# iris1997jiatong/I-DCCRN-VAE

Hardware: AMD Instinct MI355X
Metric: 4s@16kHz utterances/sec fwd+SI-SNR, DCCRN-CL, 1/2/4/8 MI355X vs host CPU (higher is better)
Workload: dtype f32; 1 GPU; supervised DCCRN-CL forward(train=False) + final_ete_loss (weights 0/0/1); batch_per_gpu=64, utterance=4 s @ 16 kHz (64000 samples, 641 frames), parallelism=replicas x1, streams=1, input=resident in HBM

## Files before the change

i-dccrn-vae_amd/csrc/cgemm_tw.hip:

```cpp
#include <atomic>
#include <cstdint>
#include <cstdlib>
#include <type_traits>
#include "cgemm.hpp"
#include "../../include/idccrn_hip.h"

namespace {

struct TwArgs {
    const float* x0;
    const float* x1;
    int C0, C1;
    int Fin, Fout;
    int J, Jp, Tp;
    const float* wfrag;
    int UP;
    const float* epi;
    int has_fold;
    const float* slope;
    float* out;
    int Cout, cotiles;
    int tshift, t_valid;
    double* stats;
    int stats_rep;
    const float* add;
    int add_div, add_Jp;
    int jtiles, ftiles;
    int xcd_split;
    int cgroups;
    int stagger;
};

constexpr int TW_PACK_CI = 8;
constexpr int TW_WVEC_MASK = 1;
constexpr int TW_XCD_SPLIT = 1;
constexpr int TW_PAIR_STAGGER = 1;

template <int PH> __device__ __forceinline__ int tw_ra(int r) {
    if (PH == 0) return r == 0 ? 0 : (r == 2 ? 2 : 1);
    return r == 0 ? 1 : 2;
}
template <int PH> __device__ __forceinline__ int tw_rb(int r) {
    if (PH == 0) return r == 2 ? 1 : (r == 3 ? 3 : 2);
    return r == 0 ? 2 : 3;
}
template <int PH> __device__ __forceinline__ float tw_cb(int r) {
    if (PH == 0) return r == 1 ? 1.f : -1.f;
    return r == 1 ? 0.f : -1.f;
}
template <int PH> constexpr int tw_nr() { return PH == 0 ? 4 : 3; }
template <int PH> constexpr int tw_nt() { return tw_nr<PH>() * 9; }
template <int PH> constexpr int tw_ntp() { return PH == 0 ? 36 : 32; }
template <int PH> constexpr int tw_ntw() { return (tw_nt<PH>() + 3) / 4; }
__host__ __device__ inline int tw_tile(int ph, int w, int k) {
    if (ph == 0) return w * 9 + k;
    if (w < 3) return k < 6 ? w * 9 + k : w * 9 + 8;
    return k < 6 ? (k >> 1) * 9 + 6 + (k & 1) : -1;
}
template <int PH> constexpr int tw_wslots() { return PH == 0 ? 9 : 8; }

template <int PH, int CIK, bool LEFT, bool STATS = false, int NCT = 1>
__global__ __launch_bounds__(256 * NCT, NCT == 1 ? 2 : 1) void cconv_tw_kernel(const TwArgs a) {
    constexpr int NR = tw_nr<PH>(), NT = tw_nt<PH>(), NTP = tw_ntp<PH>(), NTW = tw_ntw<PH>();
    constexpr int NRAW = PH == 0 ? 4 : 3, ROW0 = PH == 0 ? 0 : 1;
    constexpr int KS = CIK / 2;
    constexpr int RT = NRAW * 9 * 32;
    constexpr int NE = CIK * RT;
    constexpr int NBUF = 2;
    constexpr int RDW = 2;
    constexpr bool WVEC = (TW_WVEC_MASK >> PH) & 1;
    constexpr int NITEM = CIK * NRAW * 16;
    constexpr int NTHR = 256 * NCT;
    constexpr int NLD = (NITEM + NTHR - 1) / NTHR;
    static_assert(NCT == 1 || NCT == 2, "one or two co tiles per workgroup");
    static_assert(KS % RDW == 0 && NLD <= 2, "weight ring slots are compile-time; at most two staging items per thread");
    static_assert(NLD + NCT - 1 < KS, "the staging k-steps (from 1 on, waves 4 .. 7 one later) end before the barrier's k-step");
    static_assert(NCT * NT * 4 * 64 <= NBUF * NE, "the epilogue exchange (one area per co tile) fits the patch buffers");

    extern __shared__ __attribute__((aligned(16))) float smem[];

    const int tid = threadIdx.x;
    const int lane = tid & 63;
    const int wave = __builtin_amdgcn_readfirstlane(tid >> 6);
    const int w4 = NCT == 1 ? wave : wave & 3, cth = NCT == 1 ? 0 : wave >> 2;
    const int half = lane >> 5, l31 = lane & 31;

    const int bid = blockIdx.x;
    const int xcd = bid & 7, slot = bid >> 3;
    int jt, ft, ct;
    if (a.xcd_split) {
        const int G = 8 / a.cgroups;
        ct = xcd % a.cgroups;
        jt = (slot / a.ftiles) * G + xcd / a.cgroups;
        ft = slot - (slot / a.ftiles) * a.ftiles;
    } else {
        const int per = a.cgroups * a.ftiles;
        jt = (slot / per) * 8 + xcd;
        const int rem = slot - (slot / per) * per;
        ft = rem / a.cgroups;
        ct = rem - ft * a.cgroups;
    }
    if (jt >= a.jtiles) return;
    ct = NCT * ct + cth;
    const int j0 = jt * 64;
    const int m0 = 2 * ft;
    const int rbase = m0 - 1 + ROW0;

    const int Cin = a.C0 + a.C1;
    const int nchunk = (Cin + CIK - 1) / CIK;

    f32x16 acc[NTW];
#pragma unroll
    for (int k = 0; k < NTW; ++k)
#pragma unroll
        for (int r = 0; r < 16; ++r) acc[k][r] = 0.f;
    constexpr int NPAIR = (NTW - 1) / 2;
    constexpr bool UNI = PH == 0;
    int offA[UNI ? 1 : NPAIR + 1], offB[UNI ? 1 : NPAIR + 1];
    float cbj[UNI ? 1 : NPAIR + 1];
    if (UNI) {
        cbj[0] = tw_cb<PH>(w4);
        offA[0] = (tw_ra<PH>(w4) - ROW0) * 288;
        offB[0] = (tw_rb<PH>(w4) - ROW0) * 288;
    } else {
#pragma unroll
        for (int j = 0; j <= NPAIR; ++j) {
            int t = tw_tile(PH, w4, j < NPAIR ? 2 * j : NTW - 1);
            t = t < 0 ? 0 : t;
            const int r = t / 9, plane = t - r * 9;
            cbj[j] = tw_cb<PH>(r);
            const int po = plane == 8 ? 256 : (plane >> 1) * 64;
            offA[j] = (tw_ra<PH>(r) - ROW0) * 288 + po;
            offB[j] = cbj[j] != 0.f ? (tw_rb<PH>(r) - ROW0) * 288 + po : offA[j];
        }
    }

    f32x4 v_r[NLD], v_i[NLD];
    float e_r[NLD], e_i[NLD];
    unsigned off_v[NLD], off_e[NLD], ldsoff[NLD];
    unsigned okmask[NLD];
    int item_cl[NLD];
    bool interior[NLD];
#pragma unroll
    for (int i = 0; i < NLD; ++i) {
        const int e = tid + i * NTHR;
        const int c8 = e & 15;
        const int rl = (e >> 4) % NRAW, cl = e / (16 * NRAW);
        item_cl[i] = cl;
        const int f = rbase + rl;
        const int jc = j0 + 4 * c8;
        const int je = LEFT ? jc - 1 : jc + 4;
        const bool exists = e < NITEM;
        const bool okr = exists && f >= 0 && f < a.Fin;
        unsigned m = 0;
#pragma unroll
        for (int q = 0; q < 5; ++q) {
            const int c = jc + q + (LEFT ? -1 : 0);
            if (c >= 0 && c < a.J) m |= 1u << q;
        }
        if (okr) m |= 1u << 5;
        if (exists) m |= 1u << 7;
        const int jcv = jc + 3 < a.Jp ? jc : 0;
        const int jev = (je >= 0 && je < a.Jp) ? je : 0;
        off_v[i] = okr ? (unsigned)((cl * a.Fin + f) * a.Jp + jcv) : 0u;
        off_e[i] = okr ? (unsigned)((cl * a.Fin + f) * a.Jp + jev) : 0u;
        if (jc + 3 >= a.Jp) m &= ~0x1fu;
        if (!(je >= 0 && je < a.Jp)) m &= LEFT ? ~1u : ~(1u << 4);
        okmask[i] = m;
        interior[i] = __builtin_amdgcn_ballot_w64((m & 0xbfu) == 0xbfu) == ~0ull;
        ldsoff[i] = (unsigned)((cl * NRAW + rl) * 288 + 4 * c8);
    }
    auto stage_load = [&](int chunk, int i) {
        const int ci0 = chunk * CIK;
        const bool from0 = ci0 < a.C0;
        const float* br = from0 ? a.x0 + (size_t)ci0 * a.Fin * a.Jp : a.x1 + (size_t)(ci0 - a.C0) * a.Fin * a.Jp;
        const float* bi = from0 ? br + (size_t)a.C0 * a.Fin * a.Jp : br + (size_t)a.C1 * a.Fin * a.Jp;
        const int cvalid = (from0 ? a.C0 : Cin) - ci0;
        const bool dead = item_cl[i] >= cvalid;
        const unsigned ov = dead ? 0u : off_v[i], oe = dead ? 0u : off_e[i];
        v_r[i] = *(const f32x4*)(br + ov);
        v_i[i] = *(const f32x4*)(bi + ov);
        e_r[i] = br[oe];
        e_i[i] = bi[oe];
    };
    float fr[5], fi[5];
    auto stage_window = [&](int chunk, int i) {
        const int ci0s = chunk * CIK;
        const int cvalid = (ci0s < a.C0 ? a.C0 : Cin) - ci0s;
        constexpr bool left = LEFT;
        if (interior[i] && cvalid >= CIK) {
#pragma unroll
            for (int q = 0; q < 5; ++q) {
                fr[q] = left ? (q == 0 ? e_r[i] : v_r[i][q == 0 ? 0 : q - 1]) : (q == 4 ? e_r[i] : v_r[i][q == 4 ? 3 : q]);
                fi[q] = left ? (q == 0 ? e_i[i] : v_i[i][q == 0 ? 0 : q - 1]) : (q == 4 ? e_i[i] : v_i[i][q == 4 ? 3 : q]);
            }
            return;
        }
        unsigned m = okmask[i];
        if (item_cl[i] >= cvalid || !((m >> 5) & 1u)) m &= ~0x1fu;
#pragma unroll
        for (int q = 0; q < 5; ++q) {
            const float xr = left ? (q == 0 ? e_r[i] : v_r[i][q == 0 ? 0 : q - 1]) : (q == 4 ? e_r[i] : v_r[i][q == 4 ? 3 : q]);
            const float xi = left ? (q == 0 ? e_i[i] : v_i[i][q == 0 ? 0 : q - 1]) : (q == 4 ? e_i[i] : v_i[i][q == 4 ? 3 : q]);
            const bool cok = (m >> q) & 1u;
            fr[q] = cok ? xr : 0.f;
            fi[q] = cok ? xi : 0.f;
        }
    };
    auto plane_val = [&](int gt, int pr) -> float {
        const int g = gt / 3, tau = gt - g * 3;
        const int q0 = 2 * pr;
        const float xa_ = g == 0 ? fr[q0] + fi[q0] : (g == 1 ? fr[q0] : fi[q0]);
        const float xb_ = g == 0 ? fr[q0 + 1] + fi[q0 + 1] : (g == 1 ? fr[q0 + 1] : fi[q0 + 1]);
        const float xd_ = g == 0 ? fr[q0 + 2] + fi[q0 + 2] : (g == 1 ? fr[q0 + 2] : fi[q0 + 2]);
        return tau == 0 ? xa_ - xb_ : (tau == 1 ? xb_ : xb_ - xd_);
    };
    auto item_exists = [&](int i) -> bool { return NITEM >= (i + 1) * NTHR || wave * 64 + i * NTHR < NITEM; };
    auto stage_plane2 = [&](float* dst, int i, int j) {
        if (!item_exists(i)) return;
        if (j < 4) {
            f32x4 o = {plane_val(2 * j, 0), plane_val(2 * j + 1, 0), plane_val(2 * j, 1), plane_val(2 * j + 1, 1)};
            *(f32x4*)(dst + ldsoff[i] + j * 64) = o;
        } else {
            *(float2*)(dst + ldsoff[i] - 2 * (int)(tid & 15) + 256) = make_float2(plane_val(8, 0), plane_val(8, 1));
        }
    };
    auto stage_store = [&](float* dst, int chunk, int i) {
        stage_window(chunk, i);
#pragma unroll
        for (int j = 0; j < 5; ++j) stage_plane2(dst, i, j);
    };

    constexpr int WS = tw_wslots<PH>();
    const float* wbase = a.wfrag + ((size_t)(PH == 1 ? (size_t)a.cotiles * a.UP * tw_ntp<0>() : 0) + (size_t)ct * a.UP * NTP) * 64 +
                         (size_t)w4 * WS * 64;
    const int total_ks = nchunk * KS;
    float a_w[RDW][NTW];
    auto load_w = [&](int g, float (&dst)[NTW]) {
        g = g < total_ks ? g : total_ks - 1;
        const float* ws = wbase + (size_t)g * NTP * 64;
        if (WVEC) {
            const f32x4 w0 = *(const f32x4*)(ws + lane * 4), w1 = *(const f32x4*)(ws + 256 + lane * 4);
#pragma unroll
            for (int k = 0; k < 4; ++k) {
                dst[k] = w0[k];
                if (4 + k < NTW) dst[4 + k] = w1[k];
            }
            if (NTW == 9) dst[NTW - 1] = ws[512 + lane];
        } else {
#pragma unroll
            for (int k = 0; k < NTW; ++k) dst[k] = ws[k * 64 + lane];
        }
    };
    float xa[NTW], xb[NTW];
    auto load_raw2 = [&](const float* base, int j) {
        if (j < NPAIR) {
            const int oa = UNI ? offA[0] + j * 64 : offA[UNI ? 0 : j], ob = UNI ? offB[0] + j * 64 : offB[UNI ? 0 : j];
            const float2 pa_ = *(const float2*)(base + oa + 2 * l31), pb_ = *(const float2*)(base + ob + 2 * l31);
            xa[2 * j] = pa_.x; xa[2 * j + 1] = pa_.y;
            xb[2 * j] = pb_.x; xb[2 * j + 1] = pb_.y;
        } else {
            xa[NTW - 1] = base[(UNI ? offA[0] + 256 : offA[UNI ? 0 : NPAIR]) + l31];
            xb[NTW - 1] = base[(UNI ? offB[0] + 256 : offB[UNI ? 0 : NPAIR]) + l31];
        }
    };
    auto load_raw_all = [&](const float* base) {
#pragma unroll
        for (int j = 0; j <= NPAIR; ++j) load_raw2(base, j);
    };

#pragma unroll
    for (int i = 0; i < NLD; ++i) stage_load(0, i);
#pragma unroll
    for (int u = 0; u < RDW; ++u) load_w(u, a_w[u]);
#pragma unroll
    for (int i = 0; i < NLD; ++i) stage_store(smem, 0, i);
#pragma unroll
    for (int i = 0; i < NLD; ++i) stage_load(nchunk > 1 ? 1 : 0, i);
    __syncthreads();

    load_raw_all(smem + (size_t)half * RT);
    auto run = [&](auto late_) {
        constexpr bool LATE = decltype(late_)::value;
        for (int chunk = 0; chunk < nchunk; ++chunk) {
            const float* P = smem + (chunk & 1) * NE;
            float* Pn = smem + ((chunk + 1) & 1) * NE;
            const int nxt = chunk + 1 < nchunk ? chunk + 1 : chunk, nxt2 = chunk + 2 < nchunk ? chunk + 2 : nchunk - 1;
#pragma unroll
            for (int ul = 0; ul < KS; ++ul) {
                const float* bnext = ul + 1 < KS ? P + (size_t)(2 * (ul + 1) + half) * RT : Pn + (size_t)half * RT;
                const int si = ul - 1 - (LATE ? 1 : 0);
                const bool staging = si >= 0 && si < NLD;
#pragma unroll
                for (int k = 0; k < NTW; ++k) {
                    const float b = xa[k] + cbj[UNI ? 0 : (k >> 1 < NPAIR ? k >> 1 : NPAIR)] * xb[k];
                    acc[k] = __builtin_amdgcn_mfma_f32_32x32x2f32(a_w[ul % RDW][k], b, acc[k], 0, 0, 0);
                    if (ul == KS - 1 && k == 0) {
                        __builtin_amdgcn_sched_barrier(0);
                        __syncthreads();
                    }
                    if ((k & 1) && (k >> 1) < NPAIR) load_raw2(bnext, k >> 1);
                    if (k == NTW - 1) load_raw2(bnext, NPAIR);
                    if (staging) {
                        if (k == 0) stage_window(nxt, si);
                        if ((k & 1) && k < 6) stage_plane2(Pn, si, k >> 1);
                        if (k == (NTW == 9 ? 7 : 6)) stage_plane2(Pn, si, 3);
                        if (k == NTW - 1) stage_plane2(Pn, si, 4);
                        if (k == NTW - 1) stage_load(nxt2, si);
                    }
                    __builtin_amdgcn_sched_barrier(0);
                }
                load_w(chunk * KS + ul + RDW, a_w[ul % RDW]);
            }
        }
    };
    if (NCT == 2 && PH == 1 && a.stagger && cth)
        run(std::integral_constant<bool, NCT == 2 && PH == 1>{});
    else
        run(std::false_type{});
    __syncthreads();

    const float slope = a.slope ? *a.slope : 1.0f;
    const bool has_act = a.slope != nullptr;
    float* E = smem + cth * (NT * 4 * 64);
    const int jA = j0 + 2 * l31;
    bool keep[2], inb[2];
    int ja[2];
#pragma unroll
    for (int q = 0; q < 2; ++q) {
        const int j = jA + q;
        const int bj = j / a.Tp, tp = j - bj * a.Tp;
        inb[q] = j < a.J;
        keep[q] = inb[q] && tp >= 1 && tp <= a.t_valid;
        ja[q] = j - (bj - bj / a.add_div) * a.Tp;
    }
#pragma unroll
    for (int s = 0; s < 4; ++s) {
        if (s > 0) __syncthreads();
#pragma unroll
        for (int k = 0; k < NTW; ++k) {
            const int t = tw_tile(PH, w4, k);
            if (t >= 0) {
#pragma unroll
                for (int rr = 0; rr < 4; ++rr) E[(t * 4 + rr) * 64 + lane] = acc[k][4 * s + rr];
            }
        }
        __syncthreads();
        float v[NT];
#pragma unroll
        for (int t = 0; t < NT; ++t) v[t] = E[(t * 4 + w4) * 64 + lane];
        float pr[NR][2], pi[NR][2];
#pragma unroll
        for (int r = 0; r < NR; ++r) {
            float y[3][2];
#pragma unroll
            for (int g = 0; g < 3; ++g) {
                const float m1 = v[r * 9 + g * 3], m2 = v[r * 9 + g * 3 + 1], m3 = v[r * 9 + g * 3 + 2];
                y[g][0] = m1 + m2;
                y[g][1] = m2 - m3;
            }
#pragma unroll
            for (int q = 0; q < 2; ++q) {
                pr[r][q] = y[0][q] - y[2][q];
                pi[r][q] = y[0][q] + y[1][q];
            }
        }
        const int rg = 4 * s + w4;
        const int co = ct * 32 + (rg & 3) + 8 * (rg >> 2) + 4 * half;
        const bool cok = co < a.Cout;
        const f32x4 e0 = *(const f32x4*)(a.epi + (size_t)co * 8);
        const float e4 = a.epi[(size_t)co * 8 + 4], e5 = a.epi[(size_t)co * 8 + 5];
        float st[5] = {0.f, 0.f, 0.f, 0.f, 0.f};
#pragma unroll
        for (int rt = 0; rt < 2; ++rt) {
            const int fo = 2 * m0 + PH + 2 * rt;
            if (fo >= a.Fout) continue;
            float yr[2], yi[2];
#pragma unroll
            for (int q = 0; q < 2; ++q) {
                float re, im;
                if (PH == 0) {
                    re = rt == 0 ? pr[0][q] + pr[1][q] + pr[2][q] : pr[1][q] - pr[2][q] - pr[NR - 1][q];
                    im = rt == 0 ? pi[0][q] + pi[1][q] + pi[2][q] : pi[1][q] - pi[2][q] - pi[NR - 1][q];
                } else {
                    re = rt == 0 ? pr[0][q] + pr[1][q] : pr[1][q] - pr[2][q];
                    im = rt == 0 ? pi[0][q] + pi[1][q] : pi[1][q] - pi[2][q];
                }
                if (a.add && cok && inb[q]) {
                    re += a.add[((size_t)co * a.Fout + fo) * a.add_Jp + ja[q]];
                    im += a.add[((size_t)(a.Cout + co) * a.Fout + fo) * a.add_Jp + ja[q]];
                }
                float r_, i_;
                if (a.has_fold) {
                    r_ = e0[0] * re + e0[1] * im + e4;
                    i_ = e0[2] * re + e0[3] * im + e5;
                } else {
                    r_ = re + e4;
                    i_ = im + e5;
                }
                if (has_act) {
                    r_ = r_ >= 0.f ? r_ : slope * r_;
                    i_ = i_ >= 0.f ? i_ : slope * i_;
                }
                yr[q] = keep[q] ? r_ : 0.f;
                yi[q] = keep[q] ? i_ : 0.f;
                if (STATS && keep[q]) {
                    st[0] += yr[q];
                    st[1] += yi[q];
                    st[2] += yr[q] * yr[q];
                    st[3] += yi[q] * yi[q];
                    st[4] += yr[q] * yi[q];
                }
            }
            if (cok) {
                float* o_r = a.out + ((size_t)co * a.Fout + fo) * a.Jp + jA;
                float* o_i = a.out + ((size_t)(a.Cout + co) * a.Fout + fo) * a.Jp + jA;
                if (inb[1]) {
                    *(float2*)o_r = make_float2(yr[0], yr[1]);
                    *(float2*)o_i = make_float2(yi[0], yi[1]);
                } else if (inb[0]) {
                    o_r[0] = yr[0];
                    o_i[0] = yi[0];
                }
            }
        }
        if (STATS) {
#pragma unroll
            for (int q = 0; q < 5; ++q) {
                float tsum = st[q];
#pragma unroll
                for (int o = 16; o > 0; o >>= 1) tsum += __shfl_xor(tsum, o, 64);
                if (l31 == 0 && cok)
                    atomicAdd(&a.stats[((size_t)(a.stats_rep > 1 ? (blockIdx.x & (a.stats_rep - 1)) : 0) * a.Cout + co) * 5 + q], (double)tsum);
            }
        }
    }
}

__global__ void pack_cconv_tw_kernel(const float* __restrict__ wino, int cotiles, int UN, int UP, int vec, float* __restrict__ out) {
    const long long n0 = (long long)cotiles * UP * tw_ntp<0>() * 64, n1 = (long long)cotiles * UP * tw_ntp<1>() * 64;
    for (long long idx = blockIdx.x * (long long)blockDim.x + threadIdx.x; idx < n0 + n1; idx += (long long)gridDim.x * blockDim.x) {
        const int ph = idx >= n0;
        const long long i = ph ? idx - n0 : idx;
        const int ntp = ph ? tw_ntp<1>() : tw_ntp<0>(), nt = ph ? tw_nt<1>() : tw_nt<0>();
        const int lane = (int)(i & 63);
        long long t_ = i >> 6;
        const int t = (int)(t_ % ntp); t_ /= ntp;
        const int u = (int)(t_ % UP);
        const int ct = (int)(t_ / UP);
        float val = 0.f;
        const int ws_ = ph ? tw_wslots<1>() : tw_wslots<0>();
        const int pos = t * 64 + lane, w = pos / (ws_ * 64), q = pos % (ws_ * 64);
        const bool vec_ = (vec >> ph) & 1;
        const int k = !vec_ ? q >> 6 : (q < 512 ? (q >> 8) * 4 + (q & 3) : 8);
        const int ln = !vec_ ? q & 63 : (q < 512 ? (q & 255) >> 2 : q - 512);
        const int tt = k < (ph ? 7 : 9) ? tw_tile(ph, w, k) : -1;
        const int ci = 2 * u + (ln >> 5), co = ln & 31;
        if (tt >= 0 && ci * 3 < UN) {
            const int r = tt / 9, g = (tt % 9) / 3, tau = tt % 3;
            const float* src = wino + ((((size_t)ph * cotiles + ct) * UN + (size_t)ci * 3 + g) * 4 + r) * 64;
            const float w0 = src[co], w1 = src[32 + co];
            val = tau == 0 ? w0 : (tau == 1 ? w0 + w1 : w1);
        }
        out[idx] = val;
    }
}

template <int PH, int CIK, bool LEFT, bool STATS, int NCT>
int launch_tw_ph_l(const TwArgs& a, hipStream_t st) {
    constexpr int NE = CIK * (PH == 0 ? 4 : 3) * 9 * 32;
    constexpr size_t smem = 2 * NE * sizeof(float);
    static_assert(smem * (NCT == 1 ? 2 : 1) <= 160 * 1024, "the patch buffers of two workgroups (NCT = 2: of one) must fit the 160 KB of LDS");
    TwArgs b = a;
    b.jtiles = (a.J + 63) / 64;
    b.ftiles = PH == 1 ? a.Fin / 2 : (a.Fin + 1) / 2;
    if (b.ftiles == 0) return IDV_OK;
    b.cgroups = b.cotiles / NCT;
    if (b.cgroups * NCT != b.cotiles) return IDV_EINVAL;
    b.stagger = TW_PAIR_STAGGER;
    b.xcd_split = (TW_XCD_SPLIT && (b.cgroups == 2 || b.cgroups == 4 || b.cgroups == 8)) ? 1 : 0;
    long long nblk = (long long)((b.jtiles + 7) / 8) * 8 * b.ftiles * b.cgroups;
    if (b.xcd_split) {
        const int G = 8 / b.cgroups;
        nblk = (long long)((b.jtiles + G - 1) / G) * b.ftiles * 8;
    }
    if (nblk > 0x7fffffffLL) return IDV_EINVAL;
    auto k = cconv_tw_kernel<PH, CIK, LEFT, STATS, NCT>;
    static std::atomic<bool> attr_set[64];
    int dev = 0;
    if (hipGetDevice(&dev) != hipSuccess || dev < 0 || dev >= 64) return IDV_ELAUNCH;
    if (smem > 64 * 1024 && !attr_set[dev].load(std::memory_order_acquire)) {
        if (hipFuncSetAttribute((const void*)k, hipFuncAttributeMaxDynamicSharedMemorySize, (int)smem) != hipSuccess) return IDV_ELAUNCH;
        attr_set[dev].store(true, std::memory_order_release);
    }
    hipLaunchKernelGGL(k, dim3((unsigned)nblk), dim3(256 * NCT), smem, st, b);
    if (NCT > 1) idv_tw_pair_note_launch();
    return idv_launch_status();
}

template <int PH, int CIK>
int launch_tw_ph(const TwArgs& a, hipStream_t st) {
    const bool pair = a.cotiles % 2 == 0 && ((idv_tw_pair(-1) >> PH) & 1);
    switch ((a.stats ? 4 : 0) | (pair ? 2 : 0) | (a.tshift ? 1 : 0)) {
        case 0: return launch_tw_ph_l<PH, CIK, false, false, 1>(a, st);
        case 1: return launch_tw_ph_l<PH, CIK, true, false, 1>(a, st);
        case 2: return launch_tw_ph_l<PH, CIK, false, false, 2>(a, st);
        case 3: return launch_tw_ph_l<PH, CIK, true, false, 2>(a, st);
        case 4: return launch_tw_ph_l<PH, CIK, false, true, 1>(a, st);
        case 5: return launch_tw_ph_l<PH, CIK, true, true, 1>(a, st);
        case 6: return launch_tw_ph_l<PH, CIK, false, true, 2>(a, st);
        default: return launch_tw_ph_l<PH, CIK, true, true, 2>(a, st);
    }
}

}

namespace {
std::atomic<int>& tw_pair_mask() {
    static std::atomic<int> v{[] { const char* e = getenv("IDV_TW_PAIR"); return e ? atoi(e) & IDV_TW_PAIR_ALL : IDV_TW_PAIR_DEFAULT; }()};
    return v;
}
std::atomic<long long> tw_pair_launches{0};
}
void idv_tw_pair_note_launch() { tw_pair_launches.fetch_add(1, std::memory_order_relaxed); }
extern "C" int idv_tw_pair(int mask) {
    if (mask < 0) return tw_pair_mask().load(std::memory_order_relaxed);
    return tw_pair_mask().exchange(mask & IDV_TW_PAIR_ALL, std::memory_order_relaxed);
}
extern "C" long long idv_tw_pair_launches(int reset) {
    return reset ? tw_pair_launches.exchange(0, std::memory_order_relaxed) : tw_pair_launches.load(std::memory_order_relaxed);
}

extern "C" int idv_cconv_tw_supported(int C0, int C1, int Cout, int Fin) {
    static const int min_cout = [] { const char* e = getenv("IDV_TW_MIN_COUT"); return e ? atoi(e) : 32; }();
    if (Cout < min_cout || Fin < 2) return 0;
    if (!idv_cconv_gauss_supported(C0, C1, Cout)) return 0;
    return (C1 == 0 || C0 % 8 == 0) ? 1 : 0;
}

extern "C" long long idv_cconv_tw_wfrag_floats(int Cout, int cin_used) {
    const long long cotiles = (Cout + 31) / 32, cpad = (cin_used + TW_PACK_CI - 1) / TW_PACK_CI * TW_PACK_CI;
    return cotiles * (cpad / 2) * (36 + 32) * 64;
}

extern "C" int idv_pack_cconv_tw(const float* wino_frag, int Cout, int cin_used, float* tw_frag, void* stream) {
    if (!wino_frag || !tw_frag || Cout <= 0 || cin_used <= 0) return IDV_EINVAL;
    const int cotiles = (Cout + 31) / 32;
    const int cpad = (cin_used + TW_PACK_CI - 1) / TW_PACK_CI * TW_PACK_CI;
    const long long n = idv_cconv_tw_wfrag_floats(Cout, cin_used);
    const unsigned blocks = (unsigned)((n + 255) / 256 > 4096 ? 4096 : (n + 255) / 256);
    hipLaunchKernelGGL(pack_cconv_tw_kernel, dim3(blocks), dim3(256), 0, (hipStream_t)stream, wino_frag, cotiles, cpad * 3, cpad / 2,
                       TW_WVEC_MASK, tw_frag);
    return idv_launch_status();
}

extern "C" int idv_ctconv2d_tw_fwd(const float* x0, int C0, const float* x1, int C1, const float* wfrag, const float* epi, int has_fold,
                                   const float* prelu_slope, float* out, double* stats, double* stats_work, int stats_rep, int tshift,
                                   int Cout, int Fin, int B, int Tp, int Jp, int t_valid_out, const float* addend, int addend_div,
                                   int addend_Jp, void* stream) {
    if (!x0 || !wfrag || !epi || !out || C0 <= 0 || Cout <= 0 || Fin <= 0 || B <= 0 || Tp <= 1) return IDV_EINVAL;
    if (stats && stats_work && (stats_rep < 2 || (stats_rep & (stats_rep - 1)))) return IDV_EINVAL;
    if (addend && (addend_div < 1 || B % addend_div || addend_Jp < (B / addend_div) * Tp)) return IDV_EINVAL;
    if (C1 > 0 && !x1) return IDV_EINVAL;
    if (tshift != 0 && tshift != -1) return IDV_EINVAL;
    if (!idv_cconv_tw_supported(C0, C1, Cout, Fin)) return IDV_EINVAL;
    if ((Jp & 3) || (reinterpret_cast<uintptr_t>(x0) & 15) || (C1 > 0 && (reinterpret_cast<uintptr_t>(x1) & 15)) ||
        (reinterpret_cast<uintptr_t>(out) & 7))
        return IDV_EINVAL;
    TwArgs a{};
    a.x0 = x0; a.x1 = x1; a.C0 = C0; a.C1 = C1;
    a.Fin = Fin; a.Fout = 2 * Fin - 1;
    a.J = B * Tp; a.Jp = Jp; a.Tp = Tp;
    a.wfrag = wfrag; a.UP = (C0 + C1 + TW_PACK_CI - 1) / TW_PACK_CI * TW_PACK_CI / 2;
    a.epi = epi; a.has_fold = has_fold; a.slope = prelu_slope; a.out = out;
    a.Cout = Cout; a.cotiles = (Cout + 31) / 32;
    a.tshift = tshift; a.t_valid = t_valid_out;
    a.add = addend; a.add_div = addend ? addend_div : 1; a.add_Jp = addend_Jp;
    if (Jp < a.J) return IDV_EINVAL;
    if ((long long)8 * Fin * (long long)Jp >= 0xffffffffLL) return IDV_EINVAL;
    hipStream_t st = (hipStream_t)stream;
    a.stats = stats;
    if (stats && stats_work) { a.stats = stats_work; a.stats_rep = stats_rep; }
    int rc = 0;
    rc = launch_tw_ph<0, 8>(a, st);
    if (!rc) rc = launch_tw_ph<1, 8>(a, st);
    if (rc || !(stats && stats_work)) return rc;
    return idv_launch_stats_collapse(stats_work, stats_rep, Cout * 5, stats, st);
}
```

Baseline: 951.9 utterances/sec.

## Handle odd-Fin edge row with dedicated edge tiles in transposed complex conv

Result: faster. 973.7 utterances/sec (median of 6 runs) (+2.3%).

```diff
diff --git a/i-dccrn-vae_amd/csrc/cgemm_tw.hip b/i-dccrn-vae_amd/csrc/cgemm_tw.hip
--- a/i-dccrn-vae_amd/csrc/cgemm_tw.hip
+++ b/i-dccrn-vae_amd/csrc/cgemm_tw.hip
@@ -3,6 +3,7 @@
 #include <cstdlib>
 #include <type_traits>
 #include "cgemm.hpp"
+#include "cgemm_tw_map.hpp"
 #include "../../include/idccrn_hip.h"
 
 namespace {
@@ -25,9 +26,7 @@
     int stats_rep;
     const float* add;
     int add_div, add_Jp;
-    int jtiles, ftiles;
-    int xcd_split;
-    int cgroups;
+    TwGrid grid;
     int stagger;
 };
 
@@ -85,22 +84,11 @@
     const int w4 = NCT == 1 ? wave : wave & 3, cth = NCT == 1 ? 0 : wave >> 2;
     const int half = lane >> 5, l31 = lane & 31;
 
-    const int bid = blockIdx.x;
-    const int xcd = bid & 7, slot = bid >> 3;
-    int jt, ft, ct;
-    if (a.xcd_split) {
-        const int G = 8 / a.cgroups;
-        ct = xcd % a.cgroups;
-        jt = (slot / a.ftiles) * G + xcd / a.cgroups;
-        ft = slot - (slot / a.ftiles) * a.ftiles;
-    } else {
-        const int per = a.cgroups * a.ftiles;
-        jt = (slot / per) * 8 + xcd;
-        const int rem = slot - (slot / per) * per;
-        ft = rem / a.cgroups;
-        ct = rem - ft * a.cgroups;
-    }
-    if (jt >= a.jtiles) return;
+    TwTile tile;
+    if (!tw_block_tile(a.grid, blockIdx.x, tile)) return;
+    const bool edge = PH == 0 && tile.edge;
+    const int jt = tile.jt, ft = tile.ft;
+    int ct = tile.ct;
     ct = NCT * ct + cth;
     const int j0 = jt * 64;
     const int m0 = 2 * ft;
@@ -119,9 +107,9 @@
     int offA[UNI ? 1 : NPAIR + 1], offB[UNI ? 1 : NPAIR + 1];
     float cbj[UNI ? 1 : NPAIR + 1];
     if (UNI) {
-        cbj[0] = tw_cb<PH>(w4);
-        offA[0] = (tw_ra<PH>(w4) - ROW0) * 288;
-        offB[0] = (tw_rb<PH>(w4) - ROW0) * 288;
+        cbj[0] = edge ? 0.f : tw_cb<PH>(w4);
+        offA[0] = (edge ? w4 : tw_ra<PH>(w4) - ROW0) * 288;
+        offB[0] = (edge ? w4 : tw_rb<PH>(w4) - ROW0) * 288;
     } else {
 #pragma unroll
         for (int j = 0; j <= NPAIR; ++j) {
@@ -147,8 +135,8 @@
         const int c8 = e & 15;
         const int rl = (e >> 4) % NRAW, cl = e / (16 * NRAW);
         item_cl[i] = cl;
-        const int f = rbase + rl;
-        const int jc = j0 + 4 * c8;
+        const int f = edge ? a.Fin - 2 + (rl & 1) : rbase + rl;
+        const int jc = j0 + (edge ? 64 * (rl >> 1) : 0) + 4 * c8;
         const int je = LEFT ? jc - 1 : jc + 4;
         const bool exists = e < NITEM;
         const bool okr = exists && f >= 0 && f < a.Fin;
@@ -232,8 +220,8 @@
     };
 
     constexpr int WS = tw_wslots<PH>();
-    const float* wbase = a.wfrag + ((size_t)(PH == 1 ? (size_t)a.cotiles * a.UP * tw_ntp<0>() : 0) + (size_t)ct * a.UP * NTP) * 64 +
-                         (size_t)w4 * WS * 64;
+    const size_t wregion = PH == 1 ? (size_t)a.cotiles * a.UP * tw_ntp<0>() : (edge ? (size_t)a.cotiles * a.UP * (tw_ntp<0>() + tw_ntp<1>()) : 0);
+    const float* wbase = a.wfrag + (wregion + (size_t)ct * a.UP * NTP) * 64 + (size_t)w4 * WS * 64;
     const int total_ks = nchunk * KS;
     float a_w[RDW][NTW];
     auto load_w = [&](int g, float (&dst)[NTW]) {
@@ -323,17 +311,19 @@
     const float slope = a.slope ? *a.slope : 1.0f;
     const bool has_act = a.slope != nullptr;
     float* E = smem + cth * (NT * 4 * 64);
-    const int jA = j0 + 2 * l31;
-    bool keep[2], inb[2];
-    int ja[2];
-#pragma unroll
-    for (int q = 0; q < 2; ++q) {
-        const int j = jA + q;
-        const int bj = j / a.Tp, tp = j - bj * a.Tp;
-        inb[q] = j < a.J;
-        keep[q] = inb[q] && tp >= 1 && tp <= a.t_valid;
-        ja[q] = j - (bj - bj / a.add_div) * a.Tp;
-    }
+    const int jAc[2] = {j0 + 2 * l31, j0 + 2 * l31 + (edge ? 64 : 0)};
+    bool keep[2][2], inb[2][2];
+    int ja[2][2];
+#pragma unroll
+    for (int c = 0; c < 2; ++c)
+#pragma unroll
+        for (int q = 0; q < 2; ++q) {
+            const int j = jAc[c] + q;
+            const int bj = j / a.Tp, tp = j - bj * a.Tp;
+            inb[c][q] = j < a.J;
+            keep[c][q] = inb[c][q] && tp >= 1 && tp <= a.t_valid;
+            ja[c][q] = j - (bj - bj / a.add_div) * a.Tp;
+        }
 #pragma unroll
     for (int s = 0; s < 4; ++s) {
         if (s > 0) __syncthreads();
@@ -373,7 +363,8 @@
         float st[5] = {0.f, 0.f, 0.f, 0.f, 0.f};
 #pragma unroll
         for (int rt = 0; rt < 2; ++rt) {
-            const int fo = 2 * m0 + PH + 2 * rt;
+            const int fo = edge ? a.Fout - 1 : 2 * m0 + PH + 2 * rt;
+            const int jA = jAc[rt];
             if (fo >= a.Fout) continue;
             float yr[2], yi[2];
 #pragma unroll
@@ -382,13 +373,17 @@
                 if (PH == 0) {
                     re = rt == 0 ? pr[0][q] + pr[1][q] + pr[2][q] : pr[1][q] - pr[2][q] - pr[NR - 1][q];
                     im = rt == 0 ? pi[0][q] + pi[1][q] + pi[2][q] : pi[1][q] - pi[2][q] - pi[NR - 1][q];
+                    if (edge) {
+                        re = pr[2 * rt][q] + pr[(2 * rt + 1) % NR][q];
+                        im = pi[2 * rt][q] + pi[(2 * rt + 1) % NR][q];
+                    }
                 } else {
                     re = rt == 0 ? pr[0][q] + pr[1][q] : pr[1][q] - pr[2][q];
                     im = rt == 0 ? pi[0][q] + pi[1][q] : pi[1][q] - pi[2][q];
                 }
-                if (a.add && cok && inb[q]) {
-                    re += a.add[((size_t)co * a.Fout + fo) * a.add_Jp + ja[q]];
-                    im += a.add[((size_t)(a.Cout + co) * a.Fout + fo) * a.add_Jp + ja[q]];
+                if (a.add && cok && inb[rt][q]) {
+                    re += a.add[((size_t)co * a.Fout + fo) * a.add_Jp + ja[rt][q]];
+                    im += a.add[((size_t)(a.Cout + co) * a.Fout + fo) * a.add_Jp + ja[rt][q]];
                 }
                 float r_, i_;
                 if (a.has_fold) {
@@ -402,9 +397,9 @@
                     r_ = r_ >= 0.f ? r_ : slope * r_;
                     i_ = i_ >= 0.f ? i_ : slope * i_;
                 }
-                yr[q] = keep[q] ? r_ : 0.f;
-                yi[q] = keep[q] ? i_ : 0.f;
-                if (STATS && keep[q]) {
+                yr[q] = keep[rt][q] ? r_ : 0.f;
+                yi[q] = keep[rt][q] ? i_ : 0.f;
+                if (STATS && keep[rt][q]) {
                     st[0] += yr[q];
                     st[1] += yi[q];
                     st[2] += yr[q] * yr[q];
@@ -415,10 +410,10 @@
             if (cok) {
                 float* o_r = a.out + ((size_t)co * a.Fout + fo) * a.Jp + jA;
                 float* o_i = a.out + ((size_t)(a.Cout + co) * a.Fout + fo) * a.Jp + jA;
-                if (inb[1]) {
+                if (inb[rt][1]) {
                     *(float2*)o_r = make_float2(yr[0], yr[1]);
                     *(float2*)o_i = make_float2(yi[0], yi[1]);
-                } else if (inb[0]) {
+                } else if (inb[rt][0]) {
                     o_r[0] = yr[0];
                     o_i[0] = yi[0];
                 }
@@ -439,9 +434,10 @@
 
 __global__ void pack_cconv_tw_kernel(const float* __restrict__ wino, int cotiles, int UN, int UP, int vec, float* __restrict__ out) {
     const long long n0 = (long long)cotiles * UP * tw_ntp<0>() * 64, n1 = (long long)cotiles * UP * tw_ntp<1>() * 64;
-    for (long long idx = blockIdx.x * (long long)blockDim.x + threadIdx.x; idx < n0 + n1; idx += (long long)gridDim.x * blockDim.x) {
-        const int ph = idx >= n0;
-        const long long i = ph ? idx - n0 : idx;
+    for (long long idx = blockIdx.x * (long long)blockDim.x + threadIdx.x; idx < n0 + n1 + n0; idx += (long long)gridDim.x * blockDim.x) {
+        const bool raw = idx >= n0 + n1;
+        const int ph = idx >= n0 && !raw;
+        const long long i = raw ? idx - n0 - n1 : (ph ? idx - n0 : idx);
         const int ntp = ph ? tw_ntp<1>() : tw_ntp<0>(), nt = ph ? tw_nt<1>() : tw_nt<0>();
         const int lane = (int)(i & 63);
         long long t_ = i >> 6;
@@ -458,8 +454,12 @@
         const int ci = 2 * u + (ln >> 5), co = ln & 31;
         if (tt >= 0 && ci * 3 < UN) {
             const int r = tt / 9, g = (tt % 9) / 3, tau = tt % 3;
-            const float* src = wino + ((((size_t)ph * cotiles + ct) * UN + (size_t)ci * 3 + g) * 4 + r) * 64;
-            const float w0 = src[co], w1 = src[32 + co];
+            const float* src = wino + ((((size_t)ph * cotiles + ct) * UN + (size_t)ci * 3 + g) * 4 + (raw ? 0 : r)) * 64;
+            float w0 = src[co], w1 = src[32 + co];
+            if (raw && (r & 1)) {
+                w0 = src[64 + co] - src[128 + co];
+                w1 = src[64 + 32 + co] - src[128 + 32 + co];
+            }
             val = tau == 0 ? w0 : (tau == 1 ? w0 + w1 : w1);
         }
         out[idx] = val;
@@ -472,18 +472,11 @@
     constexpr size_t smem = 2 * NE * sizeof(float);
     static_assert(smem * (NCT == 1 ? 2 : 1) <= 160 * 1024, "the patch buffers of two workgroups (NCT = 2: of one) must fit the 160 KB of LDS");
     TwArgs b = a;
-    b.jtiles = (a.J + 63) / 64;
-    b.ftiles = PH == 1 ? a.Fin / 2 : (a.Fin + 1) / 2;
-    if (b.ftiles == 0) return IDV_OK;
-    b.cgroups = b.cotiles / NCT;
-    if (b.cgroups * NCT != b.cotiles) return IDV_EINVAL;
+    if (b.cotiles % NCT) return IDV_EINVAL;
+    b.grid = tw_grid(PH, a.Fin, a.J, b.cotiles / NCT, TW_XCD_SPLIT);
     b.stagger = TW_PAIR_STAGGER;
-    b.xcd_split = (TW_XCD_SPLIT && (b.cgroups == 2 || b.cgroups == 4 || b.cgroups == 8)) ? 1 : 0;
-    long long nblk = (long long)((b.jtiles + 7) / 8) * 8 * b.ftiles * b.cgroups;
-    if (b.xcd_split) {
-        const int G = 8 / b.cgroups;
-        nblk = (long long)((b.jtiles + G - 1) / G) * b.ftiles * 8;
-    }
+    const long long nblk = tw_grid_blocks(b.grid);
+    if (nblk == 0) return IDV_OK;
     if (nblk > 0x7fffffffLL) return IDV_EINVAL;
     auto k = cconv_tw_kernel<PH, CIK, LEFT, STATS, NCT>;
     static std::atomic<bool> attr_set[64];
@@ -540,7 +533,7 @@
 
 extern "C" long long idv_cconv_tw_wfrag_floats(int Cout, int cin_used) {
     const long long cotiles = (Cout + 31) / 32, cpad = (cin_used + TW_PACK_CI - 1) / TW_PACK_CI * TW_PACK_CI;
-    return cotiles * (cpad / 2) * (36 + 32) * 64;
+    return cotiles * (cpad / 2) * (36 + 32 + 36) * 64;
 }
 
 extern "C" int idv_pack_cconv_tw(const float* wino_frag, int Cout, int cin_used, float* tw_frag, void* stream) {
diff --git a/i-dccrn-vae_amd/csrc/cgemm_tw_map.hpp b/i-dccrn-vae_amd/csrc/cgemm_tw_map.hpp
--- /dev/null
+++ b/i-dccrn-vae_amd/csrc/cgemm_tw_map.hpp
@@ -0,0 +1,64 @@
+#pragma once
+
+#if defined(__HIPCC__) || defined(__CUDACC__)
+#define TW_HD __host__ __device__
+#else
+#define TW_HD
+#endif
+
+struct TwGrid {
+    int jtiles;
+    int ftiles;
+    int etiles;
+    int cgroups;
+    int xcd_split;
+};
+
+struct TwTile {
+    int jt, ft, ct;
+    bool edge;
+};
+
+TW_HD inline TwGrid tw_grid(int ph, int Fin, int J, int cgroups, int want_split) {
+    TwGrid g;
+    g.jtiles = (J + 63) / 64;
+    g.ftiles = Fin / 2;
+    g.etiles = (ph == 0 && (Fin & 1)) ? (g.jtiles + 1) / 2 : 0;
+    g.cgroups = cgroups;
+    g.xcd_split = (want_split && (cgroups == 2 || cgroups == 4 || cgroups == 8)) ? 1 : 0;
+    return g;
+}
+
+TW_HD inline long long tw_rounds(const TwGrid& g, int cols, int rows) {
+    if (g.xcd_split) {
+        const int G = 8 / g.cgroups;
+        return (long long)((cols + G - 1) / G) * rows;
+    }
+    return (long long)((cols + 7) / 8) * rows * g.cgroups;
+}
+
+TW_HD inline long long tw_grid_blocks(const TwGrid& g) { return 8 * (tw_rounds(g, g.etiles, 1) + tw_rounds(g, g.jtiles, g.ftiles)); }
+
+TW_HD inline bool tw_block_tile(const TwGrid& g, int bid, TwTile& t) {
+    const int xcd = bid & 7;
+    int slot = bid >> 3;
+    const int erounds = (int)tw_rounds(g, g.etiles, 1);
+    t.edge = slot < erounds;
+    if (!t.edge) slot -= erounds;
+    const int rows = t.edge ? 1 : g.ftiles, cols = t.edge ? g.etiles : g.jtiles;
+    int col;
+    if (g.xcd_split) {
+        const int G = 8 / g.cgroups;
+        t.ct = xcd % g.cgroups;
+        col = (slot / rows) * G + xcd / g.cgroups;
+        t.ft = slot - (slot / rows) * rows;
+    } else {
+        const int per = g.cgroups * rows;
+        col = (slot / per) * 8 + xcd;
+        const int rem = slot - (slot / per) * per;
+        t.ft = rem / g.cgroups;
+        t.ct = rem - t.ft * g.cgroups;
+    }
+    t.jt = t.edge ? 2 * col : col;
+    return col < cols;
+}
```
